# vliu15/3d-brain-tumor-segmentation

Measured on AMD Instinct MI355X. Metric: training volumes/sec (2ch x 128^3), higher is better.
Workload: dtype f32; 1 GPU; BASELINE configs[1]: 2ch x 128^3, batch 1 per GPU, fp32, full fwd+bwd with Dice+KL+L2 VAE loss + Dice metric + TF-form Adam; CLI-default model (base_filters=32, depth=4, groups=8, reduction=8; 42,174,773 params); parallelism=dp1, global_batch=1

## Files before the change

### 3d-brain-tumor-segmentation_amd/csrc/conv_igemm.hip

```cpp
#include <stdlib.h>
#include "common.h"
#include "conv_plan.h"

#define MAXSLOT 8

int bts_prof_on();
void bts_prof_begin(int sym, double flops, hipStream_t stream);
void bts_prof_end(hipStream_t stream);

struct IgemmParams {
  const float* x;
  const float* wp;
  const float* bias;
  float* y;
  int N, Di, Hi, Wi, Cin, ldx;
  int Do, Ho, Wo;
  int Cout, ldy, Npad, KG;
  int ODa, OHa, OWa;
  int os, ooz, ooy, oox;
  int s, loz, loy, lox;
  int IZ, IY, IX;
  int lgTX, lgTY, TZ;
  int ntz, nty, ntx;
  int ntaps, flags;
// ... 1578 lines not shown
  }
  if (c.geo == GEO_K1 && !c.second && k1s_accept(c, ch)) { ch.kernel = CONV_K1S; return BTS_OK; }
  if (c.geo == GEO_UP && !c.second && upm_accept(c, ch)) { ch.kernel = CONV_UPM; return BTS_OK; }
  ch.kernel = CONV_IGEMM;
  return igemm_accept(c, ch);
}

static int conv_launch(const ConvCall& c, const ConvChoice& ch, const ConvPtrs& q, hipStream_t stream) {
  const unsigned bit = c.geo != GEO_S1 ? 0u : ch.kernel == CONV_W3 ? 4u : ch.kernel == CONV_WINO ? 2u : 1u;
  if (bit) { const int e = bts_img_ensure_(q.wp, bit, stream); if (e != BTS_OK) return e; }
  int r;
  switch (ch.kernel) {
    case CONV_DSC: r = launch_dsc(c, ch, q, stream); break;
    case CONV_C2: r = launch_c2(c, ch, q, stream); break;
    case CONV_W3: r = bts_w3_launch_(c, ch, q, stream); break;
    case CONV_WINO: r = bts_wino_launch_(c, ch, q, stream); break;
    case CONV_K1S: r = launch_k1s(c, ch, q, stream); break;
    case CONV_UPM: r = launch_upm(c, ch, q, stream); break;
    default: r = launch_igemm(c, ch, q, stream); break;
  }
  if (r == BTS_OK && bit) bts_img_mark_used_(q.wp, bit);
  return r;
}
static int conv_run(ConvCall c, const ConvPtrs& q, hipStream_t stream, long* gn_B = nullptr) {
  auto al16 = [](const void* a) { return (((uintptr_t)a) & 15) == 0; };
  c.x16 = al16(q.x); c.y16 = al16(q.y); c.p2_16 = al16(c.second == CONV_Y2 ? (const void*)q.y2 : (const void*)q.x2); c.ws16 = al16(q.ws);
  if (q.ws == nullptr || c.ws_bytes < 0) c.ws_bytes = 0;
  if (gn_B) *gn_B = 0;
  ConvChoice ch, ch2;
  int r = conv_choose(c, ch);
  if (r != BTS_OK) return r;
  ConvCall c2 = c;
  ConvPtrs q2 = {};
  if (ch.second) {
    c2.geo = GEO_K1; c2.second = c2.G = 0; c2.ws_bytes = 0;
    if (ch.second == CONV_Y2) {
      c2.ldy = c.ld2; c2.y16 = c.p2_16; c2.flags = q.bias2 ? IG_FLAG_BIAS : 0;
      q2.x = q.x; q2.wp = q.wp2; q2.bias = q.bias2; q2.y = q.y2;
    } else {
      c2.ldx = c.ld2; c2.x16 = c.p2_16; c2.flags = IG_FLAG_ACCUM;
      q2.x = q.x2; q2.wp = q.wp2; q2.y = q.y;
    }
    r = conv_choose(c2, ch2);
    if (r != BTS_OK) return r;
  }
  r = conv_launch(c, ch, q, stream);
  if (r == BTS_OK && ch.second) r = conv_launch(c2, ch2, q2, stream);
  if (r == BTS_OK && gn_B) *gn_B = ch.gn_B;
  return r;
}

static int conv_call_of(int dir, int kind, int N, int D, int H, int W, int Cin, int ldx, int Cout, int ldy, int flags, ConvCall& c) {
  if (N <= 0 || D <= 0 || H <= 0 || W <= 0 || Cin <= 0 || Cout <= 0 || ldx < Cin || ldy < Cout) return BTS_ERR_SHAPE;
  if (kind == BTS_CONV_K3S2 && ((D | H | W) & 1)) return BTS_ERR_SHAPE;
  const bool same = kind == BTS_CONV_K1 || kind == BTS_CONV_K3S1, half = kind == BTS_CONV_K3S2;
  const int Df = same ? D : half ? D / 2 : 2 * D, Hf = same ? H : half ? H / 2 : 2 * H, Wf = same ? W : half ? W / 2 : 2 * W;
  c = ConvCall{};
  c.geo = kind == BTS_CONV_K1 ? GEO_K1 : kind == BTS_CONV_K3S1 ? GEO_S1 : half == (dir == 0) ? GEO_DOWN : GEO_UP;
  c.N = N;
  if (dir == 0) { c.Di = D; c.Hi = H; c.Wi = W; c.Do = Df; c.Ho = Hf; c.Wo = Wf; c.Cin = Cin; c.ldx = ldx; c.Cout = Cout; c.ldy = ldy; }
  else { c.Di = Df; c.Hi = Hf; c.Wi = Wf; c.Do = D; c.Ho = H; c.Wo = W; c.Cin = Cout; c.ldx = ldy; c.Cout = Cin; c.ldy = ldx; }
  if ((flags & BTS_CONV_FLAG_SIGMOID) && dir == 0) c.flags |= IG_FLAG_SIGMOID;
  if (flags & BTS_CONV_FLAG_ACCUM) c.flags |= IG_FLAG_ACCUM;
  return BTS_OK;
}
static void conv_query_view(ConvCall& c) { c.x16 = c.y16 = c.p2_16 = c.ws16 = 1; c.ws_bytes = LONG_MAX; }
static long conv_ws_query(int dir, int kind, int N, int D, int H, int W, int Cin, int Cout) {
// ... 124 lines not shown
extern "C" long bts_conv3d_bwd_data_pair_workspace(int N, int D, int H, int W, int Cin, int Cout) {
  const long a = bts_conv3d_bwd_data_workspace(BTS_CONV_K3S1, N, D, H, W, Cin, Cout);
  const long b = bts_conv3d_bwd_data_workspace(BTS_CONV_K1, N, D, H, W, Cin, Cout);
  if (a < 0 || b < 0) return -1;
  return a > b ? a : b;
}
extern "C" int bts_conv3d_bwd_data_pair(const float* dy, const float* wp_bwd, const float* dy2, const float* wp2_bwd, float* dx,
                                        void* workspace, long workspace_bytes, int N, int D, int H, int W, int Cin, int lddx,
                                        int Cout, int lddy, int lddy2, int flags, hipStream_t stream) {
  ConvCall c;
  if (conv_call_of(1, BTS_CONV_K3S1, N, D, H, W, Cin, lddx, Cout, lddy, flags, c) != BTS_OK || lddy2 < Cout) return BTS_ERR_SHAPE;
  const long need = conv_ws_query(1, BTS_CONV_K3S1, N, D, H, W, Cin, Cout);
  if (need < 0) return BTS_ERR_SHAPE;
  c.ws_bytes = workspace_bytes;
  ConvPtrs q = {};
  q.x = dy; q.wp = wp_bwd; q.y = dx; q.ws = workspace;
  const bool fuse = need == 0 && (Cout % 8 == 0) && (lddy2 % 4 == 0) && ((((uintptr_t)dy2) & 15) == 0) && Cin > 4 &&
                    getenv("BTS_IGEMM_NOPAIR") == nullptr;
  if (fuse) {
    c.second = CONV_X2; c.ld2 = lddy2;
    q.x2 = dy2; q.wp2 = wp2_bwd;
    return conv_run(c, q, stream);
  }
  const int r = conv_run(c, q, stream);
  if (r != BTS_OK) return r;
  return bts_conv3d_bwd_data(BTS_CONV_K1, dy2, wp2_bwd, dx, workspace, workspace_bytes, N, D, H, W, Cin, lddx, Cout, lddy2,
                             flags | BTS_CONV_FLAG_ACCUM, stream);
}

static int conv_config_query(int dir, int kind, int N, int D, int H, int W, int Cin, int Cout) {
  ConvCall c;
  ConvChoice ch;
  int r = conv_call_of(dir, kind, N, D, H, W, Cin, Cin, Cout, Cout, 0, c);
  if (r != BTS_OK) return r;
  conv_query_view(c);
  r = igemm_accept(c, ch);
  return r != BTS_OK ? r : ch.sym;
}
extern "C" int bts_conv3d_fwd_config(int kind, int N, int D, int H, int W, int Cin, int Cout) {
  return conv_config_query(0, kind, N, D, H, W, Cin, Cout);
}
extern "C" int bts_conv3d_bwd_data_config(int kind, int N, int D, int H, int W, int Cin, int Cout) {
  return conv_config_query(1, kind, N, D, H, W, Cin, Cout);
}
extern "C" int bts_conv3d_kernel(int dir, int kind, int N, int D, int H, int W, int Cin, int ldx, int Cout, int ldy, int flags, int second,
                                 int ld2, int G, int aligned, long workspace_bytes) {
// ... 13 lines not shown
```

### 3d-brain-tumor-segmentation_amd/csrc/loss.hip

```cpp
#include "common.h"
#include "bts_internal.h"

#define LOSS_MAXC 8
#define LOSS_BLOCKS 1024

__global__ __launch_bounds__(256) void loss_partial_kernel(const float* __restrict__ ypred, const float* __restrict__ y,
                                                           const float* __restrict__ x, const float* __restrict__ yvae,
                                                           double* partial, long NV, int C, int ldp, int ldy, int Cx,
                                                           int ldx, int ldv) {
  __shared__ double sh[8];
  double acc[3 * LOSS_MAXC + 1];
#pragma unroll
  for (int i = 0; i < 3 * LOSS_MAXC + 1; ++i) acc[i] = 0.0;
  for (long v = blockIdx.x * (long)blockDim.x + threadIdx.x; v < NV; v += (long)gridDim.x * blockDim.x) {
#pragma unroll
    for (int c = 0; c < LOSS_MAXC; ++c)
      if (c < C) {
        const float p = ypred[v * ldp + c], t = y[v * ldy + c];
        acc[c] += (double)(p * t);
        acc[LOSS_MAXC + c] += (double)(p * p);
        acc[2 * LOSS_MAXC + c] += (double)(t * t);
      }
    if (x) {
      float m = 0.f;
      for (int c = 0; c < Cx; ++c) {
        const float d = x[v * ldx + c] - yvae[v * ldv + c];
        m = fmaf(d, d, m);
      }
      acc[3 * LOSS_MAXC] += (double)m;
    }
  }
  for (int i = 0; i < 3 * LOSS_MAXC + 1; ++i) {
    const double r = block_sum_f64(acc[i], sh);
    if (threadIdx.x == 0) partial[(long)blockIdx.x * (3 * LOSS_MAXC + 1) + i] = r;
  }
}

__global__ void loss_sums_finalize_kernel(const double* partial, const float* proj, double* sums, int blocks, int C, int N,
                                          int Lz, double numel_x) {
  __shared__ double sh[8];
  for (int i = 0; i < 3 * C + 1; ++i) {
    const int src = (i < 3 * C) ? (i / C) * LOSS_MAXC + (i % C) : 3 * LOSS_MAXC;
    double s = 0.0;
    for (int b = threadIdx.x; b < blocks; b += blockDim.x) s += partial[(long)b * (3 * LOSS_MAXC + 1) + src];
    const double r = block_sum_f64(s, sh);
    if (threadIdx.x == 0) sums[i] = r;
  }
  double k = 0.0;
  if (proj)
    for (int i = threadIdx.x; i < N * Lz; i += blockDim.x) {
      const int n = i / Lz, j = i % Lz;
      const float mu = proj[n * 2 * Lz + j], lv = proj[n * 2 * Lz + Lz + j];
      k += (double)(mu * mu + expf(lv) - lv - 1.0f);
    }
  const double rk = block_sum_f64(k, sh);
  if (threadIdx.x == 0) {
    sums[3 * C + 1] = rk;
    sums[3 * C + 2] = numel_x;
    sums[3 * C + 3] = (double)N * Lz;
  }
}

extern "C" long bts_loss_workspace(void) { return (long)LOSS_BLOCKS * (3 * LOSS_MAXC + 1) * 8 + 64; }

extern "C" int bts_loss_sums(const float* y_pred, const float* y, const float* x, const float* y_vae, const float* proj,
                             double* sums, void* workspace, long workspace_bytes, int N, long V, int C, int ldp, int ldy,
                             int Cx, int ldx, int ldv, int Lz, hipStream_t stream) {
  if (N <= 0 || V <= 0 || C <= 0 || C > LOSS_MAXC) return BTS_ERR_SHAPE;
  if (workspace_bytes < bts_loss_workspace()) return BTS_ERR_WORKSPACE;
  const long NV = (long)N * V;
  long blocks = (NV + 255) / 256;
  if (blocks > LOSS_BLOCKS) blocks = LOSS_BLOCKS;
  double* partial = reinterpret_cast<double*>(workspace);
  (void)hipGetLastError(); hipLaunchKernelGGL(loss_partial_kernel, dim3((int)blocks), dim3(256), 0, stream, y_pred, y, x, y_vae, partial, NV, C, ldp,
                     ldy, Cx, ldx, ldv);
  BTS_LAUNCH_CHECK();
  (void)hipGetLastError(); hipLaunchKernelGGL(loss_sums_finalize_kernel, dim3(1), dim3(256), 0, stream, partial, proj, sums, (int)blocks, C, N, Lz,
                     (double)NV * Cx);
  BTS_LAUNCH_CHECK();
  return BTS_OK;
}

__global__ void loss_value_kernel(const double* sums, float* loss, float* parts, int C, int has_vae) {
  if (threadIdx.x || blockIdx.x) return;
  double d = 0.0;
  for (int c = 0; c < C; ++c) d += 1.0 - (2.0 * sums[c] + 1.0) / (sums[C + c] + sums[2 * C + c] + 1.0);
  d /= C;
  double l2 = 0.0, kl = 0.0;
  if (has_vae) {
    l2 = sums[3 * C] / sums[3 * C + 2];
    kl = sums[3 * C + 1] / sums[3 * C + 3];
  }
  loss[0] = (float)(d + 0.1 * l2 + 0.1 * kl);
  if (parts) { parts[0] = (float)d; parts[1] = (float)l2; parts[2] = (float)kl; }
}
extern "C" int bts_loss_value(const double* sums, float* loss, float* parts, int C, int has_vae, hipStream_t stream) {
  (void)hipGetLastError(); hipLaunchKernelGGL(loss_value_kernel, dim3(1), dim3(64), 0, stream, sums, loss, parts, C, has_vae);
  BTS_LAUNCH_CHECK();
  return BTS_OK;
}

__global__ __launch_bounds__(256) void loss_bwd_kernel(const float* __restrict__ ypred, const float* __restrict__ y,
                                                       const float* __restrict__ x, const float* __restrict__ yvae,
                                                       const float* __restrict__ proj, const double* __restrict__ sums,
                                                       const float* __restrict__ gscale, float* __restrict__ dlogit,
                                                       float* __restrict__ dyvae, float* __restrict__ dproj, long NV, int C,
                                                       int ldp, int ldy, int Cx, int ldx, int ldv, int N, int Lz,
                                                       int through_sigmoid) {
  const float gs = gscale ? gscale[0] : 1.f;
  float k1[LOSS_MAXC], k2[LOSS_MAXC];
#pragma unroll
  for (int c = 0; c < LOSS_MAXC; ++c) {
    k1[c] = k2[c] = 0.f;
    if (c < C) {
      const double D = sums[C + c] + sums[2 * C + c] + 1.0;
      k1[c] = (float)(-2.0 / (C * D) * gs);
      k2[c] = (float)(2.0 * (2.0 * sums[c] + 1.0) / (C * D * D) * gs);
    }
  }
  const float kx = x ? (float)(0.2 / sums[3 * C + 2]) * gs : 0.f;
  for (long v = blockIdx.x * (long)blockDim.x + threadIdx.x; v < NV; v += (long)gridDim.x * blockDim.x) {
#pragma unroll
    for (int c = 0; c < LOSS_MAXC; ++c)
      if (c < C) {
        const float p = ypred[v * ldp + c], t = y[v * ldy + c];
        float g = k1[c] * t + k2[c] * p;
        if (through_sigmoid) g *= p * (1.f - p);
        dlogit[v * C + c] = g;
      }
    if (x)
      for (int c = 0; c < Cx; ++c) dyvae[v * Cx + c] = kx * (yvae[v * ldv + c] - x[v * ldx + c]);
  }
  if (proj && blockIdx.x == 0) {
    const float kz = (float)(1.0 / sums[3 * C + 3]) * gs;
    for (int i = threadIdx.x; i < N * Lz; i += blockDim.x) {
      const int n = i / Lz, j = i % Lz;
      dproj[n * 2 * Lz + j] = 0.2f * kz * proj[n * 2 * Lz + j];
      dproj[n * 2 * Lz + Lz + j] = 0.1f * kz * (expf(proj[n * 2 * Lz + Lz + j]) - 1.f);
    }
  }
}
extern "C" int bts_loss_bwd(const float* y_pred, const float* y, const float* x, const float* y_vae, const float* proj,
                            const double* sums, const float* gscale, float* dlogit, float* dyvae, float* dproj, int N, long V,
                            int C, int ldp, int ldy, int Cx, int ldx, int ldv, int Lz, int through_sigmoid,
                            hipStream_t stream) {
  if (N <= 0 || V <= 0 || C <= 0 || C > LOSS_MAXC) return BTS_ERR_SHAPE;
  const long NV = (long)N * V;
  long blocks = (NV + 255) / 256;
  if (blocks > 4096) blocks = 4096;
  (void)hipGetLastError(); hipLaunchKernelGGL(loss_bwd_kernel, dim3((int)blocks), dim3(256), 0, stream, y_pred, y, x, y_vae, proj, sums, gscale, dlogit,
                     dyvae, dproj, NV, C, ldp, ldy, Cx, ldx, ldv, N, Lz, through_sigmoid);
  BTS_LAUNCH_CHECK();
  return BTS_OK;
}

__global__ void zero_f64_kernel(double* p, int n) {
  for (int i = blockIdx.x * blockDim.x + threadIdx.x; i < n; i += gridDim.x * blockDim.x) p[i] = 0.0;
}
__global__ __launch_bounds__(256) void dice_metric_kernel(const float* __restrict__ ytrue, const float* __restrict__ ypred,
                                                          uint8_t* __restrict__ labels, double* table, long NV, int C,
                                                          int ldt, int ldp, int cells, int W) {
  extern __shared__ double tab[];
  const int tsz = cells * C * 3;
  for (int i = threadIdx.x; i < tsz; i += blockDim.x) tab[i] = 0.0;
  __syncthreads();
  for (long v = blockIdx.x * (long)blockDim.x + threadIdx.x; v < NV; v += (long)gridDim.x * blockDim.x) {
    float best = ypred[v * ldp];
    int arg = 0;
    for (int c = 1; c < C; ++c) {
      const float p = ypred[v * ldp + c];
      if (p > best) { best = p; arg = c; }
    }
    const bool on = best > 0.5f;
    if (labels) labels[v] = on ? (uint8_t)(arg + 1) : 0;
    const int cell = (cells > 1) ? (int)(v % W) : 0;
    for (int c = 0; c < C; ++c) {
// ... 7 lines not shown
      if (t != 0.f) atomicAdd(e + 2, (double)t);
    }
  }
  __syncthreads();
  for (int i = threadIdx.x; i < tsz; i += blockDim.x)
    if (tab[i] != 0.0) atomicAdd(table + i, tab[i]);
}
extern "C" int bts_dice_metric_sums(const float* y_true, const float* y_pred, uint8_t* labels, double* table, int N, long V,
                                    int W, int C, int ldt, int ldp, int channels_last_axes, hipStream_t stream) {
  if (N <= 0 || V <= 0 || C <= 0 || W <= 0 || V % W) return BTS_ERR_SHAPE;
  const int cells = channels_last_axes ? W : 1;
  const int tsz = cells * C * 3;
  if ((size_t)tsz * 8 > 60 * 1024) return BTS_ERR_UNSUPPORTED;
  (void)hipGetLastError(); hipLaunchKernelGGL(zero_f64_kernel, dim3((tsz + 255) / 256), dim3(256), 0, stream, table, tsz);
  BTS_LAUNCH_CHECK();
  const long NV = (long)N * V;
  long blocks = (NV + 255) / 256;
  if (blocks > 1024) blocks = 1024;
  (void)hipGetLastError(); hipLaunchKernelGGL(dice_metric_kernel, dim3((int)blocks), dim3(256), tsz * sizeof(double), stream, y_true, y_pred, labels,
                     table, NV, C, ldt, ldp, cells, W);
  BTS_LAUNCH_CHECK();
  return BTS_OK;
}
__global__ void dice_metric_value_kernel(const double* table, float* out, int cells, int C) {
  if (blockIdx.x || threadIdx.x >= 64) return;
  double macro = 0.0, si = 0.0, sp = 0.0, st = 0.0;
  for (int i = threadIdx.x; i < cells * C; i += 64) {
    const double I = table[i * 3], P = table[i * 3 + 1], T = table[i * 3 + 2];
    macro += (2.0 * I + 1.0) / (P + T + 1.0);
    si += I; sp += P; st += T;
  }
  macro = wave_sum_f64(macro); si = wave_sum_f64(si); sp = wave_sum_f64(sp); st = wave_sum_f64(st);
  if (threadIdx.x == 0) {
    out[0] = (float)(macro / (cells * C));
    out[1] = (float)(si / (sp + st));
  }
}
extern "C" int bts_dice_metric_value(const double* table, float* out, int W, int C, int channels_last_axes,
                                     hipStream_t stream) {
  (void)hipGetLastError(); hipLaunchKernelGGL(dice_metric_value_kernel, dim3(1), dim3(64), 0, stream, table, out, channels_last_axes ? W : 1, C);
  BTS_LAUNCH_CHECK();
  return BTS_OK;
}

#define L2_MAXR 128
struct L2Ranges {
  long off[L2_MAXR], len[L2_MAXR];
  float coef[L2_MAXR];
  int nr;
};
__global__ __launch_bounds__(256) void l2_partial_kernel(const float* __restrict__ p, double* partial, L2Ranges rg) {
  __shared__ double sh[8];
  double acc = 0.0;
  for (int r = 0; r < rg.nr; ++r) {
    const float* q = p + rg.off[r];
    double s = 0.0;
    for (long i = blockIdx.x * (long)blockDim.x + threadIdx.x; i < rg.len[r]; i += (long)gridDim.x * blockDim.x)
      s += (double)(q[i] * q[i]);
    acc += (double)rg.coef[r] * s;
// ... 49 lines not shown
```

### 3d-brain-tumor-segmentation_amd/model.py

```python
import numpy as np
import torch

from . import ops, parallel
from .layers._base import Layer, Tensor, as_tensor, check_data_format, current_tape, mark_public_layout, to_internal
from .layers.decoder import Decoder
from .layers.encoder import Encoder
from .layers.vae import VariationalAutoencoder
from .tape import bump_weights_epoch


class Model(Layer):
    def __init__(self, data_format='channels_last', groups=8, reduction=2, l2_scale=1e-5, dropout=0.2,
                 downsampling='conv', upsampling='conv', base_filters=16, depth=4, in_ch=2, out_ch=3):
        super(Model, self).__init__(name='model')
        self.data_format = check_data_format(data_format)
        self.epoch = _EpochVariable()
        self.in_ch = in_ch
        self.encoder = self.track(Encoder(data_format=data_format, groups=groups, reduction=reduction, l2_scale=l2_scale,
                                          dropout=dropout, downsampling=downsampling, base_filters=base_filters,
                                          depth=depth, _reserve_for_decoder=True))
        self.decoder = self.track(Decoder(data_format=data_format, groups=groups, reduction=reduction, l2_scale=l2_scale,
                                          upsampling=upsampling, base_filters=base_filters, depth=depth, out_ch=out_ch))
        self.vae = self.track(VariationalAutoencoder(data_format=data_format, groups=groups, reduction=reduction,
                                                     l2_scale=l2_scale, upsampling=upsampling,
                                                     base_filters=base_filters, depth=depth, out_ch=in_ch))
        self.flat_params = None
        self.flat_grads = None
        self._l2_ranges = None

    def build(self, input_shape):
        shp = tuple(input_shape)
# ... 52 lines not shown
                    if (p.l2 if p.l2 > 0 else 0.0) != cls:
                        continue
                    n = p.t.numel()
                    flat[off:off + n].copy_(p.t.reshape(-1))
                    p.t = flat[off:off + n].view(p.t.shape)
                    p._gview = grads[off:off + n].view(p.t.shape)
                    off += n
                if cls > 0 and off > c0:
                    if ranges and ranges[-1][2] == cls and ranges[-1][0] + ranges[-1][1] == c0:
                        ranges[-1] = (ranges[-1][0], ranges[-1][1] + off - c0, cls)
                    else:
                        ranges.append((c0, off - c0, cls))
            spans.append((start, off))
        if len(ranges) > 128:
            raise RuntimeError('more than 128 regulariser ranges')
        self.flat_params, self.flat_grads, self._l2_ranges = flat, grads, ranges
        self._group_spans = spans
        self.n_params = total
        bump_weights_epoch()

    def call(self, inputs, training=None, inference=None):
        assert (not inference or not training), 'Cannot run training and inference modes simultaneously.'
        x = as_tensor(inputs, data_format=self.data_format)
        residuals = self.encoder(x, training=training)
        y_pred = self.decoder((residuals[-1], residuals[:-1]), training=training)
        if inference:
            return (y_pred, None, None, None)
        y_vae, z_mean, z_logvar = self.vae(residuals[-1], training=training)
        return (y_pred, y_vae, z_mean, z_logvar)

    def __call__(self, inputs, training=None, inference=None):
        cf = self.data_format == 'channels_first'
        if cf:
            inputs = to_internal(inputs)
        if not self.built:
            self.build(tuple(inputs.shape))
        out = self.call(inputs, training=training, inference=inference)
        return mark_public_layout(out) if cf else out

    @property
    def trainable_variables(self):
        return self.encoder.trainable_variables + self.decoder.trainable_variables + self.vae.trainable_variables

    @property
    def losses(self):
        if self.flat_params is None or not self._l2_ranges:
            return Layer.losses.fget(self)
        val = Tensor(ops.l2_reg_fwd(self.flat_params, self._l2_ranges))
        tape = current_tape()
        if tape is not None:
            gen = tape.gen

            self._l2_val, self._l2_val_gen = val, tape.gen

            def backward():
                g = val.grad
                if g is None:
                    return
                from .tape import current_or_replaying_tape
                tp = current_or_replaying_tape()
                if tp is not None and tp.grad_sync is not None:
                    return
                ops.join_side_stream()
                for p in self.trainable_variables:
                    if p._gen != gen:
                        ops.fill(p._gview, 0.0)
                        p._gen = gen
                k = parallel.l2_grad_scale()
                ops.l2_reg_bwd(self.flat_params, self.flat_grads, [(o, l, c * k) for o, l, c in self._l2_ranges], g)
            tape.nodes.insert(0, backward)
        return [val]
# ... 64 lines not shown
```

### 3d-brain-tumor-segmentation_amd/ops.py

```python
import ctypes
import weakref

import numpy as np
import torch

from ._lib import ERRORS, lib

K1, K3S1, K3S2, K3S2T = 0, 1, 2, 3
ROLE_FWD, ROLE_BWD = 0, 1
FLAG_SIGMOID, FLAG_ACCUM = 1, 2
GN_SLAB, GN_CHANNEL = 0, 1

_workspaces = {}

_CFG = {0: '2,1,4,1', 1: '2,2,4,1', 2: '1,2,2,2', 3: '1,1,2,2', 4: '1,1,4,1'}


_VARIANTS = {33: {1: '<0,5>', 2: '<0,4>', 3: '<1,5>', 4: '<1,4>'},
             32: {1: '<3x3x3>', 2: '<1x1x1>'}}


def kernel_symbol(sym, detail=False):
    var, sym = sym >> 16, sym & 0xffff
    if var and detail and sym in _VARIANTS:
# ... 526 lines not shown
    lib().call('bts_loss_sums', _p(y_pred), _p(y), _p(x), _p(y_vae), _p(proj), _p(sums), _p(ws), nb, n, v, c, ld_of(y_pred),
               ld_of(y), cx, ld_of(x) if has_vae else 0, ld_of(y_vae) if has_vae else 0, lz, _stream())
    return sums


def loss_value(sums, c, has_vae=True):
    loss = torch.empty(1, dtype=torch.float32, device=sums.device)
    parts = torch.empty(3, dtype=torch.float32, device=sums.device)
    lib().call('bts_loss_value', _p(sums), _p(loss), _p(parts), c, 1 if has_vae else 0, _stream())
    return loss, parts


def loss_bwd(y_pred, y, x, y_vae, proj, sums, gscale, dypred, dyvae, dproj, through_sigmoid=False):
    n, c = y_pred.shape[0], y_pred.shape[4]
    v = y_pred.shape[1] * y_pred.shape[2] * y_pred.shape[3]
    has_vae = x is not None
    cx = x.shape[4] if has_vae else 0
    lz = proj.shape[1] // 2 if proj is not None else 0
    lib().call('bts_loss_bwd', _p(y_pred), _p(y), _p(x), _p(y_vae), _p(proj), _p(sums), _p(gscale), _p(dypred), _p(dyvae),
               _p(dproj), n, v, c, ld_of(y_pred), ld_of(y), cx, ld_of(x) if has_vae else 0, ld_of(y_vae) if has_vae else 0,
               lz, 1 if through_sigmoid else 0, _stream())


def dice_metric_sums(y_true, y_pred, channels_last_axes=True, want_labels=True):
    n, d, h, w, c = y_pred.shape
    cells = w if channels_last_axes else 1
    table = torch.empty(cells * c * 3, dtype=torch.float64, device=y_pred.device)
    labels = torch.empty((n, d, h, w), dtype=torch.uint8, device=y_pred.device) if want_labels else None
    lib().call('bts_dice_metric_sums', _p(y_true), _p(y_pred), _p(labels), _p(table), n, d * h * w, w, c, ld_of(y_true),
               ld_of(y_pred), 1 if channels_last_axes else 0, _stream())
    return table, labels


def dice_metric_value(table, w, c, channels_last_axes=True):
    out = torch.empty(2, dtype=torch.float32, device=table.device)
    lib().call('bts_dice_metric_value', _p(table), _p(out), w, c, 1 if channels_last_axes else 0, _stream())
    return out


def _ranges(ranges):
    nr = len(ranges)
    off = (ctypes.c_long * max(nr, 1))(*[r[0] for r in ranges])
    ln = (ctypes.c_long * max(nr, 1))(*[r[1] for r in ranges])
    cf = (ctypes.c_float * max(nr, 1))(*[r[2] for r in ranges])
    return off, ln, cf, nr

# ... 644 lines not shown
```

### 3d-brain-tumor-segmentation_amd/util.py

```python
import math

import torch

from . import ops, parallel
from .tape import GradientTape, Tensor, as_tensor, bump_weights_epoch, current_tape


class DiceVAELoss(object):

    def __init__(self, name='custom_loss', data_format='channels_last', **kwargs):
        if data_format not in ('channels_last', 'channels_first'):
            raise ValueError('unknown data_format %r' % (data_format,))
        self.data_format = data_format
        self.axis = (0, 1, 2, 3) if data_format == 'channels_last' else (0, 2, 3, 4)

    def __call__(self, x, y, y_pred, y_vae, z_mean, z_logvar, sample_weight=None):
        x, y = as_tensor(x, data_format=self.data_format), as_tensor(y, data_format=self.data_format)
        y_pred, y_vae = as_tensor(y_pred, True), as_tensor(y_vae, True)
        pbase = getattr(z_mean, 'base', None)
        if pbase is None or pbase is not getattr(z_logvar, 'base', None):
            raise ValueError('z_mean / z_logvar must be the two halves of the VAE projection returned by Model')
        proj = pbase.t
        c = y_pred.shape[-1]
        sums = ops.loss_sums(y_pred.t, y.t, x.t, y_vae.t, proj)
        parallel.all_reduce_sum(sums)
        lt, parts = ops.loss_value(sums, c, True)
        loss = Tensor(lt)
        self.last_parts = parts
        tape = current_tape()
        if tape is not None:
            def backward():
                g = loss.grad
                if g is None:
                    return
                dyp = torch.empty(y_pred.shape, dtype=torch.float32, device=g.device)
                dyv = torch.empty(y_vae.shape, dtype=torch.float32, device=g.device)
                dpr = torch.empty_like(proj)
                ops.loss_bwd(y_pred.t, y.t, x.t, y_vae.t, proj, sums, g, dyp, dyv, dpr, through_sigmoid=False)
                for src, d in ((y_pred, dyp), (y_vae, dyv)):
                    if src.requires_grad:
                        buf, acc = src.grad_slot()
                        ops.add_strided(buf, d, acc)
                ops.axpy(pbase.grad_full(), dpr, 1.0)
            tape.record(backward)
        return loss


class DiceCoefficient(object):

    def __init__(self, name='dice_coefficient', data_format='channels_last'):
        if data_format not in ('channels_last', 'channels_first'):
            raise ValueError('unknown data_format %r' % (data_format,))
        self.name = name
        self.data_format = data_format
        self.last_labels = None

    def __call__(self, y_true, y_pred):
        y_true, y_pred = as_tensor(y_true, data_format=self.data_format), as_tensor(y_pred, data_format=self.data_format)
        w, c = y_pred.shape[3], y_pred.shape[4]
        cl = self.data_format == 'channels_last'
        table, labels = ops.dice_metric_sums(y_true.t, y_pred.t, cl, True)
        parallel.all_reduce_sum(table)
        out = ops.dice_metric_value(table, w, c, cl)
        self.last_labels = labels
        return Tensor(out[0:1], requires_grad=False), Tensor(out[1:2], requires_grad=False)


class ScheduledOptim(object):

    def __init__(self, learning_rate=1e-4, beta_1=0.9, beta_2=0.999, epsilon=1e-7, amsgrad=False, name='Adam',
                 n_epochs=300, **kwargs):
        if amsgrad:
            raise NotImplementedError('amsgrad=True is never used by the reference (util.py:65)')
        self.init_lr = float(learning_rate)
        self.learning_rate = float(learning_rate)
        self.beta_1, self.beta_2, self.epsilon = float(beta_1), float(beta_2), float(epsilon)
        self.n_epochs = float(n_epochs)
        self.iterations = 0
        self._state = {}

    def __call__(self, epoch):
        self.learning_rate = self.init_lr * ((1.0 - epoch / self.n_epochs) ** 0.9)

    def _lr_t(self):
        t = self.iterations
        return self.learning_rate * math.sqrt(1.0 - self.beta_2 ** t) / (1.0 - self.beta_1 ** t)
# ... 51 lines not shown
```

### include/bts_hip.h

```cpp
#ifndef BTS_HIP_H
#define BTS_HIP_H
#include <stdint.h>
#ifdef __cplusplus
extern "C" {
#endif

typedef struct ihipStream_t* bts_stream_t;

#define BTS_OK 0
#define BTS_ERR_SHAPE (-1)
#define BTS_ERR_ALIGN (-2)
#define BTS_ERR_UNSUPPORTED (-3)
#define BTS_ERR_WORKSPACE (-4)
#define BTS_ERR_RCCL_BASE (-100)

#define BTS_CONV_K1 0
#define BTS_CONV_K3S1 1
#define BTS_CONV_K3S2 2
#define BTS_CONV_K3S2T 3
#define BTS_ROLE_FWD 0
#define BTS_ROLE_BWD_DATA 1
#define BTS_CONV_FLAG_SIGMOID 1
#define BTS_CONV_FLAG_ACCUM 2

// ... 70 lines not shown
int bts_axpy(float* y, const float* x, long n, float a, bts_stream_t stream);
int bts_add_strided(float* dst, const float* src, long rows, int C, int ldd, int lds_, int accumulate, bts_stream_t stream);
int bts_scalar_lincomb(float* out, const float* a, const float* b, float ca, float cb, bts_stream_t stream);
int bts_relu_bwd(const float* y, const float* dy, float* dx, long n, bts_stream_t stream);
int bts_sigmoid_bwd(const float* y, const float* dy, float* dx, long rows, int C, int ldy, int lddy, bts_stream_t stream);

long bts_dense_workspace(int N, int in, int out);
int bts_dense_fwd(const float* x, const float* w, const float* bias, float* y, void* workspace, long workspace_bytes, int N,
                  int in, int out, int relu, bts_stream_t stream);
int bts_dense_bwd(const float* x, const float* w, const float* g, float* dx, float* dw, float* db, int N, int in, int out,
                  int accumulate_dx, int accumulate_params, bts_stream_t stream);

long bts_loss_workspace(void);
int bts_loss_sums(const float* y_pred, const float* y, const float* x, const float* y_vae, const float* proj, double* sums,
                  void* workspace, long workspace_bytes, int N, long V, int C, int ldp, int ldy, int Cx, int ldx, int ldv,
                  int Lz, bts_stream_t stream);
int bts_loss_value(const double* sums, float* loss, float* parts, int C, int has_vae, bts_stream_t stream);
int bts_loss_bwd(const float* y_pred, const float* y, const float* x, const float* y_vae, const float* proj,
                 const double* sums, const float* gscale, float* dlogit, float* dyvae, float* dproj, int N, long V, int C,
                 int ldp, int ldy, int Cx, int ldx, int ldv, int Lz, int through_sigmoid, bts_stream_t stream);
int bts_dice_metric_sums(const float* y_true, const float* y_pred, uint8_t* labels, double* table, int N, long V, int W,
                         int C, int ldt, int ldp, int channels_last_axes, bts_stream_t stream);
int bts_dice_metric_value(const double* table, float* out, int W, int C, int channels_last_axes, bts_stream_t stream);
long bts_l2_workspace(void);
int bts_l2_reg_fwd(const float* params, const long* off, const long* len, const float* coef, int nranges, float* out,
                   void* workspace, long workspace_bytes, bts_stream_t stream);
int bts_l2_reg_bwd(const float* params, float* grads, const long* off, const long* len, const float* coef, int nranges,
                   const float* gscale, bts_stream_t stream);

int bts_adam_tf_step(float* p, const float* g, float* m, float* v, long n, float lr_t, float beta1, float beta2, float eps,
                     float gmul, bts_stream_t stream);
int bts_grad_nonfinite(const float* g, long n, int* flag, bts_stream_t stream);
int bts_adam_tf_step_guarded(float* p, const float* g, float* m, float* v, long n, float lr_t, float beta1, float beta2, float eps,
                             float gmul, const int* skip, bts_stream_t stream);

long bts_conv3d_bwd_data_pair_workspace(int N, int D, int H, int W, int Cin, int Cout);
int bts_conv3d_bwd_data_pair(const float* dy, const float* wp_bwd, const float* dy2, const float* wp2_bwd, float* dx,
                             void* workspace, long workspace_bytes, int N, int D, int H, int W, int Cin, int lddx, int Cout,
                             int lddy, int lddy2, int flags, bts_stream_t stream);

long bts_conv3d_fwd_gn_workspace(int kind, int N, int D, int H, int W, int Cin, int Cout, int G);
int bts_conv3d_fwd_gn(int kind, const float* x, const float* wp_fwd, const float* bias, float* y, void* workspace,
                      long workspace_bytes, int N, int D, int H, int W, int Cin, int ldx, int Cout, int G, float eps, float* mean,
                      float* rstd, bts_stream_t stream);
int bts_conv3d_fwd_fused2_gn(const float* x, const float* wp_fwd, const float* bias, float* y, const float* wp2,
                             const float* bias2, float* y2, void* workspace, long workspace_bytes, int N, int D, int H, int W,
// ... 208 lines not shown
```

Baseline: 26.97 volumes/s.

## Fuse loss with Dice metric, write loss grads in place, reorder paired bwd convs

The Dice metric table and labels are now computed inside the loss partial-sum kernel, and one finalize kernel produces the loss value, the loss sums and the Dice outputs. This saves a separate pass over the predictions and several small launches. The loss backward writes or accumulates straight into the gradient slots instead of going through temporaries and add_strided. The paired backward-data conv runs the 1x1 kernel first so the 3x3 conv can accumulate on top of it. The L2 regularizer is launched early on a side stream so it overlaps with the forward pass. The main cost is extra shared-memory double atomics in the loss kernel, plus the cached-result handoff between loss and metric, which relies on object identity.

After: 27.19 volumes/s (median of 6 runs). No clear change (+0.8%).

```diff
diff --git a/3d-brain-tumor-segmentation_amd/csrc/conv_igemm.hip b/3d-brain-tumor-segmentation_amd/csrc/conv_igemm.hip
--- a/3d-brain-tumor-segmentation_amd/csrc/conv_igemm.hip
+++ b/3d-brain-tumor-segmentation_amd/csrc/conv_igemm.hip
@@ -1624,10 +1624,13 @@
   if (r == BTS_OK && bit) bts_img_mark_used_(q.wp, bit);
   return r;
 }
-static int conv_run(ConvCall c, const ConvPtrs& q, hipStream_t stream, long* gn_B = nullptr) {
+static void conv_operand_view(ConvCall& c, const ConvPtrs& q) {
   auto al16 = [](const void* a) { return (((uintptr_t)a) & 15) == 0; };
   c.x16 = al16(q.x); c.y16 = al16(q.y); c.p2_16 = al16(c.second == CONV_Y2 ? (const void*)q.y2 : (const void*)q.x2); c.ws16 = al16(q.ws);
   if (q.ws == nullptr || c.ws_bytes < 0) c.ws_bytes = 0;
+}
+static int conv_run(ConvCall c, const ConvPtrs& q, hipStream_t stream, long* gn_B = nullptr) {
+  conv_operand_view(c, q);
   if (gn_B) *gn_B = 0;
   ConvChoice ch, ch2;
   int r = conv_choose(c, ch);
@@ -1645,6 +1648,15 @@
     }
     r = conv_choose(c2, ch2);
     if (r != BTS_OK) return r;
+    if (ch.second == CONV_X2 && !(c.flags & IG_FLAG_ACCUM) && !c.G && ch2.kernel == CONV_K1S) {
+      c2.flags &= ~IG_FLAG_ACCUM;
+      r = conv_launch(c2, ch2, q2, stream);
+      if (r != BTS_OK) return r;
+      c.flags |= IG_FLAG_ACCUM;
+      r = conv_launch(c, ch, q, stream);
+      if (r == BTS_OK && gn_B) *gn_B = 0;
+      return r;
+    }
   }
   r = conv_launch(c, ch, q, stream);
   if (r == BTS_OK && ch.second) r = conv_launch(c2, ch2, q2, stream);
@@ -1815,6 +1827,26 @@
     q.x2 = dy2; q.wp2 = wp2_bwd;
     return conv_run(c, q, stream);
   }
+  if (!(c.flags & IG_FLAG_ACCUM)) {
+    ConvCall ca = c, ck;
+    ConvPtrs qk = {};
+    qk.x = dy2; qk.wp = wp2_bwd; qk.y = dx; qk.ws = workspace;
+    ConvChoice ch, cha, chk;
+    conv_operand_view(ca, q);
+    const bool plain = conv_choose(ca, ch) == BTS_OK;
+    ca.flags |= IG_FLAG_ACCUM;
+    if (plain && conv_choose(ca, cha) == BTS_OK && cha.kernel == ch.kernel && cha.sym == ch.sym && cha.ws == ch.ws &&
+        conv_call_of(1, BTS_CONV_K1, N, D, H, W, Cin, lddx, Cout, lddy2, 0, ck) == BTS_OK) {
+      ck.ws_bytes = workspace_bytes;
+      conv_operand_view(ck, qk);
+      if (conv_choose(ck, chk) == BTS_OK && chk.kernel == CONV_K1S) {
+        const int r1 = conv_run(ck, qk, stream);
+        if (r1 != BTS_OK) return r1;
+        c.flags |= IG_FLAG_ACCUM;
+        return conv_run(c, q, stream);
+      }
+    }
+  }
   const int r = conv_run(c, q, stream);
   if (r != BTS_OK) return r;
   return bts_conv3d_bwd_data(BTS_CONV_K1, dy2, wp2_bwd, dx, workspace, workspace_bytes, N, D, H, W, Cin, lddx, Cout, lddy2,
diff --git a/3d-brain-tumor-segmentation_amd/csrc/loss.hip b/3d-brain-tumor-segmentation_amd/csrc/loss.hip
--- a/3d-brain-tumor-segmentation_amd/csrc/loss.hip
+++ b/3d-brain-tumor-segmentation_amd/csrc/loss.hip
@@ -4,23 +4,54 @@
 #define LOSS_MAXC 8
 #define LOSS_BLOCKS 1024
 
+template <bool DICE>
 __global__ __launch_bounds__(256) void loss_partial_kernel(const float* __restrict__ ypred, const float* __restrict__ y,
                                                            const float* __restrict__ x, const float* __restrict__ yvae,
                                                            double* partial, long NV, int C, int ldp, int ldy, int Cx,
-                                                           int ldx, int ldv) {
+                                                           int ldx, int ldv, uint8_t* __restrict__ labels, double* table,
+                                                           int cells, int W) {
   __shared__ double sh[8];
+  extern __shared__ double tab[];
+  const int tsz = cells * C * 3;
+  if (DICE) {
+    for (int i = threadIdx.x; i < tsz; i += blockDim.x) tab[i] = 0.0;
+    __syncthreads();
+  }
   double acc[3 * LOSS_MAXC + 1];
 #pragma unroll
   for (int i = 0; i < 3 * LOSS_MAXC + 1; ++i) acc[i] = 0.0;
   for (long v = blockIdx.x * (long)blockDim.x + threadIdx.x; v < NV; v += (long)gridDim.x * blockDim.x) {
+    float pv[LOSS_MAXC], tv[LOSS_MAXC];
 #pragma unroll
     for (int c = 0; c < LOSS_MAXC; ++c)
       if (c < C) {
         const float p = ypred[v * ldp + c], t = y[v * ldy + c];
+        pv[c] = p; tv[c] = t;
         acc[c] += (double)(p * t);
         acc[LOSS_MAXC + c] += (double)(p * p);
         acc[2 * LOSS_MAXC + c] += (double)(t * t);
       }
+    if (DICE) {
+      float best = pv[0];
+      int arg = 0;
+#pragma unroll
+      for (int c = 1; c < LOSS_MAXC; ++c)
+        if (c < C && pv[c] > best) { best = pv[c]; arg = c; }
+      const bool on = best > 0.5f;
+      if (labels) labels[v] = on ? (uint8_t)(arg + 1) : 0;
+      const int cell = (cells > 1) ? (int)(v % W) : 0;
+#pragma unroll
+      for (int c = 0; c < LOSS_MAXC; ++c)
+        if (c < C) {
+          const float t = tv[c];
+          double* e = tab + (cell * C + c) * 3;
+          if (on && c == arg) {
+            atomicAdd(e + 1, 1.0);
+            if (t != 0.f) atomicAdd(e, (double)t);
+          }
+          if (t != 0.f) atomicAdd(e + 2, (double)t);
+        }
+    }
     if (x) {
       float m = 0.f;
       for (int c = 0; c < Cx; ++c) {
@@ -33,6 +64,10 @@
   for (int i = 0; i < 3 * LOSS_MAXC + 1; ++i) {
     const double r = block_sum_f64(acc[i], sh);
     if (threadIdx.x == 0) partial[(long)blockIdx.x * (3 * LOSS_MAXC + 1) + i] = r;
+  }
+  if (DICE) {
+    for (int i = threadIdx.x; i < tsz; i += blockDim.x)
+      if (tab[i] != 0.0) atomicAdd(table + i, tab[i]);
   }
 }
 
@@ -72,8 +107,8 @@
   long blocks = (NV + 255) / 256;
   if (blocks > LOSS_BLOCKS) blocks = LOSS_BLOCKS;
   double* partial = reinterpret_cast<double*>(workspace);
-  (void)hipGetLastError(); hipLaunchKernelGGL(loss_partial_kernel, dim3((int)blocks), dim3(256), 0, stream, y_pred, y, x, y_vae, partial, NV, C, ldp,
-                     ldy, Cx, ldx, ldv);
+  (void)hipGetLastError(); hipLaunchKernelGGL(loss_partial_kernel<false>, dim3((int)blocks), dim3(256), 0, stream, y_pred, y, x, y_vae, partial, NV, C, ldp,
+                     ldy, Cx, ldx, ldv, (uint8_t*)nullptr, (double*)nullptr, 0, 1);
   BTS_LAUNCH_CHECK();
   (void)hipGetLastError(); hipLaunchKernelGGL(loss_sums_finalize_kernel, dim3(1), dim3(256), 0, stream, partial, proj, sums, (int)blocks, C, N, Lz,
                      (double)NV * Cx);
@@ -81,8 +116,49 @@
   return BTS_OK;
 }
 
-__global__ void loss_value_kernel(const double* sums, float* loss, float* parts, int C, int has_vae) {
-  if (threadIdx.x || blockIdx.x) return;
+__device__ __forceinline__ void loss_value_of(const double* sums, float* loss, float* parts, int C, int has_vae);
+__device__ __forceinline__ void dice_value_of(const double* table, float* out, int cells, int C);
+
+__global__ __launch_bounds__(256) void loss_dice_finalize_kernel(const double* partial, const float* proj, double* sums, int blocks,
+                                                                 int C, int N, int Lz, double numel_x, float* loss, float* parts,
+                                                                 int has_vae, const double* table, float* dice_out, int cells) {
+  __shared__ double sh[8];
+  double s[3 * LOSS_MAXC + 1];
+#pragma unroll
+  for (int i = 0; i < 3 * LOSS_MAXC + 1; ++i) s[i] = 0.0;
+  for (int b = threadIdx.x; b < blocks; b += blockDim.x) {
+    const double* row = partial + (long)b * (3 * LOSS_MAXC + 1);
+#pragma unroll
+    for (int i = 0; i < 3 * LOSS_MAXC + 1; ++i)
+      if (i == 3 * LOSS_MAXC || (i % LOSS_MAXC) < C) s[i] += row[i];
+  }
+  for (int i = 0; i < 3 * C + 1; ++i) {
+    const int src = (i < 3 * C) ? (i / C) * LOSS_MAXC + (i % C) : 3 * LOSS_MAXC;
+    double v = 0.0;
+#pragma unroll
+    for (int j = 0; j < 3 * LOSS_MAXC + 1; ++j)
+      if (j == src) v = s[j];
+    const double r = block_sum_f64(v, sh);
+    if (threadIdx.x == 0) sums[i] = r;
+  }
+  double k = 0.0;
+  if (proj)
+    for (int i = threadIdx.x; i < N * Lz; i += blockDim.x) {
+      const int n = i / Lz, j = i % Lz;
+      const float mu = proj[n * 2 * Lz + j], lv = proj[n * 2 * Lz + Lz + j];
+      k += (double)(mu * mu + expf(lv) - lv - 1.0f);
+    }
+  const double rk = block_sum_f64(k, sh);
+  if (threadIdx.x == 0) {
+    sums[3 * C + 1] = rk;
+    sums[3 * C + 2] = numel_x;
+    sums[3 * C + 3] = (double)N * Lz;
+    if (loss) loss_value_of(sums, loss, parts, C, has_vae);
+  }
+  if (dice_out && threadIdx.x < 64) dice_value_of(table, dice_out, cells, C);
+}
+
+__device__ __forceinline__ void loss_value_of(const double* sums, float* loss, float* parts, int C, int has_vae) {
   double d = 0.0;
   for (int c = 0; c < C; ++c) d += 1.0 - (2.0 * sums[c] + 1.0) / (sums[C + c] + sums[2 * C + c] + 1.0);
   d /= C;
@@ -94,19 +170,27 @@
   loss[0] = (float)(d + 0.1 * l2 + 0.1 * kl);
   if (parts) { parts[0] = (float)d; parts[1] = (float)l2; parts[2] = (float)kl; }
 }
+__global__ void loss_value_kernel(const double* sums, float* loss, float* parts, int C, int has_vae) {
+  if (threadIdx.x || blockIdx.x) return;
+  loss_value_of(sums, loss, parts, C, has_vae);
+}
 extern "C" int bts_loss_value(const double* sums, float* loss, float* parts, int C, int has_vae, hipStream_t stream) {
   (void)hipGetLastError(); hipLaunchKernelGGL(loss_value_kernel, dim3(1), dim3(64), 0, stream, sums, loss, parts, C, has_vae);
   BTS_LAUNCH_CHECK();
   return BTS_OK;
 }
 
+__device__ __forceinline__ float add_rounded(float a, float g) {
+  asm volatile("" : "+v"(g));
+  return a + g;
+}
 __global__ __launch_bounds__(256) void loss_bwd_kernel(const float* __restrict__ ypred, const float* __restrict__ y,
                                                        const float* __restrict__ x, const float* __restrict__ yvae,
                                                        const float* __restrict__ proj, const double* __restrict__ sums,
                                                        const float* __restrict__ gscale, float* __restrict__ dlogit,
                                                        float* __restrict__ dyvae, float* __restrict__ dproj, long NV, int C,
                                                        int ldp, int ldy, int Cx, int ldx, int ldv, int N, int Lz,
-                                                       int through_sigmoid) {
+                                                       int through_sigmoid, int lddl, int lddv, int accl, int accv) {
   const float gs = gscale ? gscale[0] : 1.f;
   float k1[LOSS_MAXC], k2[LOSS_MAXC];
 #pragma unroll
@@ -126,10 +210,15 @@
         const float p = ypred[v * ldp + c], t = y[v * ldy + c];
         float g = k1[c] * t + k2[c] * p;
         if (through_sigmoid) g *= p * (1.f - p);
-        dlogit[v * C + c] = g;
+        float* o = dlogit + v * lddl + c;
+        *o = accl ? add_rounded(*o, g) : g;
       }
     if (x)
-      for (int c = 0; c < Cx; ++c) dyvae[v * Cx + c] = kx * (yvae[v * ldv + c] - x[v * ldx + c]);
+      for (int c = 0; c < Cx; ++c) {
+        const float g = kx * (yvae[v * ldv + c] - x[v * ldx + c]);
+        float* o = dyvae + v * lddv + c;
+        *o = accv ? add_rounded(*o, g) : g;
+      }
   }
   if (proj && blockIdx.x == 0) {
     const float kz = (float)(1.0 / sums[3 * C + 3]) * gs;
@@ -140,18 +229,25 @@
     }
   }
 }
+extern "C" int bts_loss_bwd_into(const float* y_pred, const float* y, const float* x, const float* y_vae, const float* proj,
+                                 const double* sums, const float* gscale, float* dlogit, float* dyvae, float* dproj, int N, long V,
+                                 int C, int ldp, int ldy, int Cx, int ldx, int ldv, int Lz, int through_sigmoid, int lddl, int lddv,
+                                 int accl, int accv, hipStream_t stream) {
+  if (N <= 0 || V <= 0 || C <= 0 || C > LOSS_MAXC || lddl < C || (x && lddv < Cx)) return BTS_ERR_SHAPE;
+  const long NV = (long)N * V;
+  long blocks = (NV + 255) / 256;
+  if (blocks > 4096) blocks = 4096;
+  (void)hipGetLastError(); hipLaunchKernelGGL(loss_bwd_kernel, dim3((int)blocks), dim3(256), 0, stream, y_pred, y, x, y_vae, proj, sums, gscale, dlogit,
+                     dyvae, dproj, NV, C, ldp, ldy, Cx, ldx, ldv, N, Lz, through_sigmoid, lddl, lddv, accl, accv);
+  BTS_LAUNCH_CHECK();
+  return BTS_OK;
+}
 extern "C" int bts_loss_bwd(const float* y_pred, const float* y, const float* x, const float* y_vae, const float* proj,
                             const double* sums, const float* gscale, float* dlogit, float* dyvae, float* dproj, int N, long V,
                             int C, int ldp, int ldy, int Cx, int ldx, int ldv, int Lz, int through_sigmoid,
                             hipStream_t stream) {
-  if (N <= 0 || V <= 0 || C <= 0 || C > LOSS_MAXC) return BTS_ERR_SHAPE;
-  const long NV = (long)N * V;
-  long blocks = (NV + 255) / 256;
-  if (blocks > 4096) blocks = 4096;
-  (void)hipGetLastError(); hipLaunchKernelGGL(loss_bwd_kernel, dim3((int)blocks), dim3(256), 0, stream, y_pred, y, x, y_vae, proj, sums, gscale, dlogit,
-                     dyvae, dproj, NV, C, ldp, ldy, Cx, ldx, ldv, N, Lz, through_sigmoid);
-  BTS_LAUNCH_CHECK();
-  return BTS_OK;
+  return bts_loss_bwd_into(y_pred, y, x, y_vae, proj, sums, gscale, dlogit, dyvae, dproj, N, V, C, ldp, ldy, Cx, ldx, ldv, Lz,
+                           through_sigmoid, C, Cx, 0, 0, stream);
 }
 
 __global__ void zero_f64_kernel(double* p, int n) {
@@ -205,8 +301,7 @@
   BTS_LAUNCH_CHECK();
   return BTS_OK;
 }
-__global__ void dice_metric_value_kernel(const double* table, float* out, int cells, int C) {
-  if (blockIdx.x || threadIdx.x >= 64) return;
+__device__ __forceinline__ void dice_value_of(const double* table, float* out, int cells, int C) {
   double macro = 0.0, si = 0.0, sp = 0.0, st = 0.0;
   for (int i = threadIdx.x; i < cells * C; i += 64) {
     const double I = table[i * 3], P = table[i * 3 + 1], T = table[i * 3 + 2];
@@ -218,6 +313,34 @@
     out[0] = (float)(macro / (cells * C));
     out[1] = (float)(si / (sp + st));
   }
+}
+__global__ void dice_metric_value_kernel(const double* table, float* out, int cells, int C) {
+  if (blockIdx.x || threadIdx.x >= 64) return;
+  dice_value_of(table, out, cells, C);
+}
+
+extern "C" int bts_loss_dice_sums(const float* y_pred, const float* y, const float* x, const float* y_vae, const float* proj,
+                                  double* sums, uint8_t* labels, double* table, float* loss, float* parts, float* dice_out,
+                                  void* workspace, long workspace_bytes, int N, long V, int W, int C, int ldp, int ldy, int Cx,
+                                  int ldx, int ldv, int Lz, int channels_last_axes, hipStream_t stream) {
+  if (N <= 0 || V <= 0 || C <= 0 || C > LOSS_MAXC || W <= 0 || V % W) return BTS_ERR_SHAPE;
+  if (workspace_bytes < bts_loss_workspace()) return BTS_ERR_WORKSPACE;
+  const int cells = channels_last_axes ? W : 1;
+  const int tsz = cells * C * 3;
+  if ((size_t)tsz * 8 > 60 * 1024) return BTS_ERR_UNSUPPORTED;
+  (void)hipGetLastError(); hipLaunchKernelGGL(zero_f64_kernel, dim3((tsz + 255) / 256), dim3(256), 0, stream, table, tsz);
+  BTS_LAUNCH_CHECK();
+  const long NV = (long)N * V;
+  long blocks = (NV + 255) / 256;
+  if (blocks > LOSS_BLOCKS) blocks = LOSS_BLOCKS;
+  double* partial = reinterpret_cast<double*>(workspace);
+  (void)hipGetLastError(); hipLaunchKernelGGL(loss_partial_kernel<true>, dim3((int)blocks), dim3(256), tsz * sizeof(double), stream, y_pred, y, x, y_vae,
+                     partial, NV, C, ldp, ldy, Cx, ldx, ldv, labels, table, cells, W);
+  BTS_LAUNCH_CHECK();
+  (void)hipGetLastError(); hipLaunchKernelGGL(loss_dice_finalize_kernel, dim3(1), dim3(256), 0, stream, partial, proj, sums, (int)blocks, C, N, Lz,
+                     (double)NV * Cx, loss, parts, (x != nullptr) ? 1 : 0, table, dice_out, cells);
+  BTS_LAUNCH_CHECK();
+  return BTS_OK;
 }
 extern "C" int bts_dice_metric_value(const double* table, float* out, int W, int C, int channels_last_axes,
                                      hipStream_t stream) {
diff --git a/3d-brain-tumor-segmentation_amd/model.py b/3d-brain-tumor-segmentation_amd/model.py
--- a/3d-brain-tumor-segmentation_amd/model.py
+++ b/3d-brain-tumor-segmentation_amd/model.py
@@ -6,7 +6,7 @@
 from .layers.decoder import Decoder
 from .layers.encoder import Encoder
 from .layers.vae import VariationalAutoencoder
-from .tape import bump_weights_epoch
+from .tape import bump_weights_epoch, weights_epoch
 
 
 class Model(Layer):
@@ -105,6 +105,9 @@
     def call(self, inputs, training=None, inference=None):
         assert (not inference or not training), 'Cannot run training and inference modes simultaneously.'
         x = as_tensor(inputs, data_format=self.data_format)
+        self._l2_early = None
+        if training:
+            self._launch_l2_early()
         residuals = self.encoder(x, training=training)
         y_pred = self.decoder((residuals[-1], residuals[:-1]), training=training)
         if inference:
@@ -125,11 +128,29 @@
     def trainable_variables(self):
         return self.encoder.trainable_variables + self.decoder.trainable_variables + self.vae.trainable_variables
 
+    def _launch_l2_early(self):
+        side = ops.side_stream('wgrad')
+        if side is None or self.flat_params is None or not self._l2_ranges or current_tape() is None:
+            return
+        cur = torch.cuda.current_stream()
+        side.wait_stream(cur)
+        with torch.cuda.stream(side):
+            val = ops.l2_reg_fwd(self.flat_params, self._l2_ranges)
+            ev = torch.cuda.Event()
+            ev.record(side)
+        val.record_stream(cur)
+        self._l2_early = (val, ev, weights_epoch())
+
     @property
     def losses(self):
         if self.flat_params is None or not self._l2_ranges:
             return Layer.losses.fget(self)
-        val = Tensor(ops.l2_reg_fwd(self.flat_params, self._l2_ranges))
+        early, self._l2_early = getattr(self, '_l2_early', None), None
+        if early is not None and early[2] == weights_epoch():
+            torch.cuda.current_stream().wait_event(early[1])
+            val = Tensor(early[0])
+        else:
+            val = Tensor(ops.l2_reg_fwd(self.flat_params, self._l2_ranges))
         tape = current_tape()
         if tape is not None:
             gen = tape.gen
diff --git a/3d-brain-tumor-segmentation_amd/ops.py b/3d-brain-tumor-segmentation_amd/ops.py
--- a/3d-brain-tumor-segmentation_amd/ops.py
+++ b/3d-brain-tumor-segmentation_amd/ops.py
@@ -572,6 +572,37 @@
                lz, 1 if through_sigmoid else 0, _stream())
 
 
+def loss_dice_sums(y_pred, y, x, y_vae, proj, channels_last_axes=True, values=True):
+    n, d, h, w, c = y_pred.shape
+    dev = y_pred.device
+    sums = torch.empty(3 * c + 4, dtype=torch.float64, device=dev)
+    table = torch.empty((w if channels_last_axes else 1) * c * 3, dtype=torch.float64, device=dev)
+    labels = torch.empty((n, d, h, w), dtype=torch.uint8, device=dev)
+    loss = torch.empty(1, dtype=torch.float32, device=dev) if values else None
+    parts = torch.empty(3, dtype=torch.float32, device=dev) if values else None
+    dice = torch.empty(2, dtype=torch.float32, device=dev) if values else None
+    nb = lib().query('bts_loss_workspace')
+    ws = workspace(nb, dev)
+    has_vae = x is not None
+    lz = proj.shape[1] // 2 if proj is not None else 0
+    lib().call('bts_loss_dice_sums', _p(y_pred), _p(y), _p(x), _p(y_vae), _p(proj), _p(sums), _p(labels), _p(table), _p(loss), _p(parts),
+               _p(dice), _p(ws), nb, n, d * h * w, w, c, ld_of(y_pred), ld_of(y), x.shape[4] if has_vae else 0,
+               ld_of(x) if has_vae else 0, ld_of(y_vae) if has_vae else 0, lz, 1 if channels_last_axes else 0, _stream())
+    return sums, table, labels, loss, parts, dice
+
+
+def loss_bwd_into(y_pred, y, x, y_vae, proj, sums, gscale, dypred, acc_pred, dyvae, acc_vae, dproj, through_sigmoid=False):
+    n, c = y_pred.shape[0], y_pred.shape[4]
+    v = y_pred.shape[1] * y_pred.shape[2] * y_pred.shape[3]
+    has_vae = x is not None
+    cx = x.shape[4] if has_vae else 0
+    lz = proj.shape[1] // 2 if proj is not None else 0
+    lib().call('bts_loss_bwd_into', _p(y_pred), _p(y), _p(x), _p(y_vae), _p(proj), _p(sums), _p(gscale), _p(dypred), _p(dyvae),
+               _p(dproj), n, v, c, ld_of(y_pred), ld_of(y), cx, ld_of(x) if has_vae else 0, ld_of(y_vae) if has_vae else 0,
+               lz, 1 if through_sigmoid else 0, ld_of(dypred), ld_of(dyvae) if has_vae else 0, 1 if acc_pred else 0,
+               1 if acc_vae else 0, _stream())
+
+
 def dice_metric_sums(y_true, y_pred, channels_last_axes=True, want_labels=True):
     n, d, h, w, c = y_pred.shape
     cells = w if channels_last_axes else 1
diff --git a/3d-brain-tumor-segmentation_amd/util.py b/3d-brain-tumor-segmentation_amd/util.py
--- a/3d-brain-tumor-segmentation_amd/util.py
+++ b/3d-brain-tumor-segmentation_amd/util.py
@@ -4,6 +4,13 @@
 
 from . import ops, parallel
 from .tape import GradientTape, Tensor, as_tensor, bump_weights_epoch, current_tape
+
+
+_fused_dice = [None]
+
+
+def _same_memory(a, b):
+    return a.data_ptr() == b.data_ptr() and a.shape == b.shape and a.stride() == b.stride()
 
 
 class DiceVAELoss(object):
@@ -22,9 +29,17 @@
             raise ValueError('z_mean / z_logvar must be the two halves of the VAE projection returned by Model')
         proj = pbase.t
         c = y_pred.shape[-1]
-        sums = ops.loss_sums(y_pred.t, y.t, x.t, y_vae.t, proj)
-        parallel.all_reduce_sum(sums)
-        lt, parts = ops.loss_value(sums, c, True)
+        single = not parallel.active()
+        cl = self.data_format == 'channels_last'
+        fused = (y_pred.shape[3] if cl else 1) * c * 3 * 8 <= 60 * 1024
+        if fused:
+            sums, table, labels, lt, parts, dice = ops.loss_dice_sums(y_pred.t, y.t, x.t, y_vae.t, proj, cl, values=single)
+            _fused_dice[0] = (y_pred, y.t, cl, table, labels, dice)
+        else:
+            sums = ops.loss_sums(y_pred.t, y.t, x.t, y_vae.t, proj)
+        if not (fused and single):
+            parallel.all_reduce_sum(sums)
+            lt, parts = ops.loss_value(sums, c, True)
         loss = Tensor(lt)
         self.last_parts = parts
         tape = current_tape()
@@ -33,14 +48,18 @@
                 g = loss.grad
                 if g is None:
                     return
-                dyp = torch.empty(y_pred.shape, dtype=torch.float32, device=g.device)
-                dyv = torch.empty(y_vae.shape, dtype=torch.float32, device=g.device)
                 dpr = torch.empty_like(proj)
-                ops.loss_bwd(y_pred.t, y.t, x.t, y_vae.t, proj, sums, g, dyp, dyv, dpr, through_sigmoid=False)
-                for src, d in ((y_pred, dyp), (y_vae, dyv)):
-                    if src.requires_grad:
-                        buf, acc = src.grad_slot()
-                        ops.add_strided(buf, d, acc)
+                if y_pred.requires_grad and y_vae.requires_grad:
+                    (dyp, accp), (dyv, accv) = y_pred.grad_slot(), y_vae.grad_slot()
+                    ops.loss_bwd_into(y_pred.t, y.t, x.t, y_vae.t, proj, sums, g, dyp, accp, dyv, accv, dpr, through_sigmoid=False)
+                else:
+                    dyp = torch.empty(y_pred.shape, dtype=torch.float32, device=g.device)
+                    dyv = torch.empty(y_vae.shape, dtype=torch.float32, device=g.device)
+                    ops.loss_bwd(y_pred.t, y.t, x.t, y_vae.t, proj, sums, g, dyp, dyv, dpr, through_sigmoid=False)
+                    for src, d in ((y_pred, dyp), (y_vae, dyv)):
+                        if src.requires_grad:
+                            buf, acc = src.grad_slot()
+                            ops.add_strided(buf, d, acc)
                 ops.axpy(pbase.grad_full(), dpr, 1.0)
             tape.record(backward)
         return loss
@@ -59,9 +78,15 @@
         y_true, y_pred = as_tensor(y_true, data_format=self.data_format), as_tensor(y_pred, data_format=self.data_format)
         w, c = y_pred.shape[3], y_pred.shape[4]
         cl = self.data_format == 'channels_last'
-        table, labels = ops.dice_metric_sums(y_true.t, y_pred.t, cl, True)
-        parallel.all_reduce_sum(table)
-        out = ops.dice_metric_value(table, w, c, cl)
+        kept, _fused_dice[0] = _fused_dice[0], None
+        out = None
+        if kept is not None and kept[0] is y_pred and kept[2] == cl and _same_memory(kept[1], y_true.t):
+            table, labels, out = kept[3:]
+        else:
+            table, labels = ops.dice_metric_sums(y_true.t, y_pred.t, cl, True)
+        if out is None:
+            parallel.all_reduce_sum(table)
+            out = ops.dice_metric_value(table, w, c, cl)
         self.last_labels = labels
         return Tensor(out[0:1], requires_grad=False), Tensor(out[1:2], requires_grad=False)
 
diff --git a/include/bts_hip.h b/include/bts_hip.h
--- a/include/bts_hip.h
+++ b/include/bts_hip.h
@@ -116,6 +116,14 @@
 int bts_dice_metric_sums(const float* y_true, const float* y_pred, uint8_t* labels, double* table, int N, long V, int W,
                          int C, int ldt, int ldp, int channels_last_axes, bts_stream_t stream);
 int bts_dice_metric_value(const double* table, float* out, int W, int C, int channels_last_axes, bts_stream_t stream);
+int bts_loss_dice_sums(const float* y_pred, const float* y, const float* x, const float* y_vae, const float* proj, double* sums,
+                       uint8_t* labels, double* table, float* loss, float* parts, float* dice_out, void* workspace,
+                       long workspace_bytes, int N, long V, int W, int C, int ldp, int ldy, int Cx, int ldx, int ldv, int Lz,
+                       int channels_last_axes, bts_stream_t stream);
+int bts_loss_bwd_into(const float* y_pred, const float* y, const float* x, const float* y_vae, const float* proj,
+                      const double* sums, const float* gscale, float* dlogit, float* dyvae, float* dproj, int N, long V, int C,
+                      int ldp, int ldy, int Cx, int ldx, int ldv, int Lz, int through_sigmoid, int lddl, int lddv, int accl,
+                      int accv, bts_stream_t stream);
 long bts_l2_workspace(void);
 int bts_l2_reg_fwd(const float* params, const long* off, const long* len, const float* coef, int nranges, float* out,
                    void* workspace, long workspace_bytes, bts_stream_t stream);
```
